# dedis/kyber

Hardware: AMD Instinct MI355X
Metric: scalar-muls/s + pairings/s per node; MSM sec at 2^20 points (higher is better)
Workload: dtype int32 limbs (radix 2^25.5), int64 accumulate; 1 GPU; Ed25519 batched fixed-base + var-base scalar-mul, 2^20 scalars per GPU (BASELINE.json configs[1]); elements_per_gpu=1048576

## Files before the change

kyber_amd/csrc/ed25519.hip:

```cpp
#ifndef KYB_TU_WAVES
#define KYB_TU_WAVES 2
#endif
#include "context.h"
#include "ed25519_dev.cuh"
#include "ed25519_launch.h"
#include "msm.cuh"
#include "ed25519_h2c.cuh"
#include <stdlib.h>
#include <string.h>

#include <algorithm>
#include <atomic>
#include <chrono>
#include <thread>
#include <vector>

namespace kyb {


template <int G = 2>
__global__ void ed25519_build_base_table_kernel(int32_t* __restrict__ tab, const uint32_t* __restrict__ point,
                                                uint32_t* __restrict__ ok, int rows = ED_TAB_POS * ED_TAB_ENT) {
    const int t = blockIdx.x * blockDim.x + threadIdx.x;
    if (t >= rows) return;
    ge_p3 B;
    if (point) {
        uint32_t pw[8];
        load_words8(pw, point);
        const bool good = ge_p3_fromwords(B, pw);
        if (t == 0) *ok = good ? 1u : 0u;
    } else {
        B.X = fe_bx(); B.Y = fe_by(); fe_1(B.Z); B.T = fe_bt();
    }
    ed_comb_row<G>(tab + (size_t)t * ED_TAB_STRIDE, t, B);
}

__global__ __launch_bounds__(64, KYB_TU_WAVES) void ed25519_encode_kernel(size_t n, const int32_t* __restrict__ proj,
                                                            const uint8_t* __restrict__ status,
                                                            uint32_t* __restrict__ out) {
    ed_encode_chunk(n, proj, (size_t)blockIdx.x * blockDim.x + threadIdx.x, [&](size_t i, uint32_t (&w)[8]) {
        if (status && status[i]) {
#pragma unroll
            for (int k = 0; k < 8; k++) w[k] = 0;
        }
        store_words8(out + i * 8, w);
    });
}


template <int G>
__global__ __launch_bounds__(256, 3) void ed25519_mul_base_kernel(
    size_t n, const uint32_t* __restrict__ scalars, uint32_t* __restrict__ out,
    const int32_t* __restrict__ tab, uint32_t flags, int32_t* __restrict__ proj) {
    const bool full = (flags & KYB_F_VARTIME) != 0;
    for (size_t idx = (size_t)blockIdx.x * blockDim.x + threadIdx.x; idx < n;
         idx += (size_t)gridDim.x * blockDim.x) {
        uint32_t a[8];
        load_words8(a, scalars + idx * 8);
        int8_t e[65];
        recode16(e, a, full);
        ge_p3 h;
        ge_p3_0(h);
        ge_precomp t;
        ge_p1p1 r;
        const int npos = full ? EdComb<G>::POS : EdComb<G>::POS_CT;
        EdCombDigits<G> digits(e);
#pragma unroll 1
        for (int k = 0; k < npos; k++) {
            const int d = digits.next(k);
            if (full && __ballot(d != 0) == 0) continue;
            select_precomp_tab<EdComb<G>::ENT>(t, tab, k, d);
            ge_madd(r, h, t);
            ge_p1p1_to_p3(h, r);
        }
        if (proj) {
            store_proj(proj, idx, h);
            continue;
        }
        uint32_t w[8];
// ... 26 lines not shown
        for (int l = 0; l < 10; l++) {
            t.ypx.v[l] ^= (t.ypx.v[l] ^ w[l]) & keep;
            t.ymx.v[l] ^= (t.ymx.v[l] ^ w[10 + l]) & keep;
            t.xy2d.v[l] ^= (t.xy2d.v[l] ^ w[20 + l]) & keep;
        }
    }
    ge_precomp_cneg(t, neg);
}
__global__ __launch_bounds__(256, 3) void ed25519_mul_base_uniform_kernel(
    size_t n, const uint32_t* __restrict__ scalars, uint32_t* __restrict__ out,
    const int32_t* __restrict__ tab, int32_t* __restrict__ proj) {
    for (size_t idx = (size_t)blockIdx.x * blockDim.x + threadIdx.x; idx < n;
         idx += (size_t)gridDim.x * blockDim.x) {
        uint32_t a[8];
        load_words8(a, scalars + idx * 8);
        int8_t e[65];
        recode16(e, a, false);
        ge_p3 h;
        ge_p3_0(h);
        ge_precomp t;
        ge_p1p1 r;
        EdCombDigits<1> digits(e);
#pragma unroll 1
        for (int i = 0; i < 64; i++) {
            select_precomp_uniform(t, tab, i, digits.next(i));
            ge_madd(r, h, t);
            ge_p1p1_to_p3(h, r);
        }
        if (proj) {
            store_proj(proj, idx, h);
            continue;
        }
        uint32_t w[8];
        ge_p3_towords(w, h);
        store_words8(out + idx * 8, w);
    }
}


template <bool GTAB, bool UNI = false>
__global__ __launch_bounds__(128, 3) void ed25519_mul_kernel(
    size_t n, const uint32_t* __restrict__ scalars, const uint32_t* __restrict__ points,
    size_t points_stride, uint32_t* __restrict__ out, uint8_t* __restrict__ status,
    uint32_t flags, int32_t* __restrict__ proj, int4* __restrict__ gtab) {
    const size_t idx = (size_t)blockIdx.x * blockDim.x + threadIdx.x;
    if (idx >= n) return;
    const bool full = !UNI && (flags & KYB_F_VARTIME) != 0;
    uint32_t pw[8], a[8];
    load_words8(pw, points + idx * points_stride);
    load_words8(a, scalars + idx * 8);
    ge_p3 A;
    const bool ok = ge_p3_fromwords(A, pw);
    int8_t e[65];
    recode16(e, a, full);
    ge_p3 h;
    const int vt_top = full ? wave_top_digit(a) : 63;
    if constexpr (GTAB) {
        TabGlobal tab{gtab + idx * 80};
        ge_scalarmult_w4<UNI, true>(h, e, A, full, tab, vt_top);
    } else {
        TabScratch tab;
        ge_scalarmult_w4<UNI, true>(h, e, A, full, tab, vt_top);
    }
    if (proj) {
        store_proj(proj, idx, h);
        if (status) status[idx] = ok ? KYB_ST_OK : KYB_ST_BAD_POINT;
        return;
    }
    uint32_t w[8];
    ge_p3_towords(w, h);
    if (!ok) {
#pragma unroll
        for (int i = 0; i < 8; i++) w[i] = 0;
    }
    store_words8(out + idx * 8, w);
    if (status) status[idx] = ok ? KYB_ST_OK : KYB_ST_BAD_POINT;
}

int ed25519_build_tables(DeviceCtx* ctx) {
    KYB_HIP_CHECK(hipMalloc(&ctx->ed_base_tab, ED_TAB_WORDS * sizeof(int32_t)));
    hipLaunchKernelGGL(ed25519_build_base_table_kernel<2>, dim3((ED_TAB_POS * ED_TAB_ENT + 63) / 64), dim3(64), 0,
                       nullptr, ctx->ed_base_tab, (const uint32_t*)nullptr, (uint32_t*)nullptr, ED_TAB_POS * ED_TAB_ENT);
    KYB_HIP_CHECK(hipGetLastError());
    const auto t0 = std::chrono::steady_clock::now();
    KYB_HIP_CHECK(hipMalloc(&ctx->ed_wide_tab, ED_WIDE_WORDS * sizeof(int32_t)));
    hipLaunchKernelGGL(ed25519_build_base_table_kernel<ED_COMB_G>, dim3((EdWide::ROWS + 63) / 64), dim3(64), 0, nullptr,
                       ctx->ed_wide_tab, (const uint32_t*)nullptr, (uint32_t*)nullptr, EdWide::ROWS);
    KYB_HIP_CHECK(hipGetLastError());
    KYB_HIP_CHECK(hipStreamSynchronize(nullptr));
    ctx->ed_wide_build_us = std::chrono::duration_cast<std::chrono::microseconds>(std::chrono::steady_clock::now() - t0).count();
    return KYB_OK;
}
void ed25519_free_tables(DeviceCtx* ctx) {
    if (ctx->ed_base_tab) hipFree(ctx->ed_base_tab);
    if (ctx->ed_wide_tab) hipFree(ctx->ed_wide_tab);
    ctx->ed_base_tab = ctx->ed_wide_tab = nullptr;
}

constexpr size_t ENC_DEFER_MIN = 4096;


static int launch_mul_base(DeviceCtx* ctx, size_t n, const void* d_scalars, void* d_out, uint32_t flags,
                           hipStream_t st, const int32_t* tab = nullptr) {
    const bool wide = !tab && !(flags & KYB_F_UNIFORM);
    if (!tab) tab = wide ? ctx->ed_wide_tab : ctx->ed_base_tab;
    if (n == 0) return KYB_OK;
    const int block = 256;
    size_t want = (n + block - 1) / block;
    size_t cap = (size_t)ctx->num_cu * 8;
    int grid = (int)(want < cap ? want : cap);
    EdSlab w{};
    std::lock_guard<std::recursive_mutex> enq_lock(ctx->enq_mu);
    if (n >= ENC_DEFER_MIN)
        if (int rc = ed_slab(ctx, st, ED_SLAB_MUL_BASE, n, &w)) return rc;
    if (flags & KYB_F_UNIFORM) {
        hipLaunchKernelGGL(ed25519_mul_base_uniform_kernel, dim3(grid), dim3(block), 0, st, n,
                           (const uint32_t*)d_scalars, (uint32_t*)d_out, tab, w.proj);
    } else {
        const auto kernel = wide ? ed25519_mul_base_kernel<ED_COMB_G> : ed25519_mul_base_kernel<2>;
        hipLaunchKernelGGL(kernel, dim3(grid), dim3(block), 0, st, n, (const uint32_t*)d_scalars, (uint32_t*)d_out, tab,
                           flags, w.proj);
    }
    if (w.proj)
        hipLaunchKernelGGL(ed25519_encode_kernel, ed_encode_grid(n), dim3(ED_ENC_BLOCK), 0, st, n, w.proj,
                           (const uint8_t*)nullptr, (uint32_t*)d_out);
    KYB_HIP_CHECK(hipGetLastError());
    return KYB_OK;
}
static int launch_mul(size_t n, const void* d_scalars, const void* d_points, size_t stride, void* d_out,
                      void* d_status, uint32_t flags, hipStream_t st) {
    if (n == 0) return KYB_OK;
    const int block = 128;
    size_t grid = (n + block - 1) / block;
    EdSlab w{};
    uint8_t* stat = (uint8_t*)d_status;
    DeviceCtx* ctx;
    int rc = get_ctx(&ctx);
    if (rc) return rc;
    std::lock_guard<std::recursive_mutex> enq_lock(ctx->enq_mu);
    const bool defer = n >= ENC_DEFER_MIN, uni = (flags & KYB_F_UNIFORM) != 0;
    const auto kernel = defer ? (uni ? ed25519_mul_kernel<true, true> : ed25519_mul_kernel<true, false>)
                              : (uni ? ed25519_mul_kernel<false, true> : ed25519_mul_kernel<false, false>);
    if (defer) {
        if ((rc = ed_slab(ctx, st, ed_slab_mul(stat == nullptr), n, &w))) return rc;
        if (!stat) stat = w.status;
    }
    hipLaunchKernelGGL(kernel, dim3((unsigned)grid), dim3(block), 0, st, n, (const uint32_t*)d_scalars,
                       (const uint32_t*)d_points, stride, (uint32_t*)d_out, stat, flags, w.proj, w.gtab);
    if (w.proj)
        hipLaunchKernelGGL(ed25519_encode_kernel, ed_encode_grid(n), dim3(ED_ENC_BLOCK), 0, st, n, w.proj,
                           (const uint8_t*)stat, (uint32_t*)d_out);
    KYB_HIP_CHECK(hipGetLastError());
    return KYB_OK;
}

}

using namespace kyb;

static bool ed_mul_flags_bad(uint32_t flags) {
    return (flags & ~(KYB_F_VARTIME | KYB_F_UNIFORM)) || (flags & (KYB_F_VARTIME | KYB_F_UNIFORM)) == (KYB_F_VARTIME | KYB_F_UNIFORM);
}

extern "C" {

int kyb_ed25519_mul_base_dev(size_t n, const void* d_scalars, void* d_out, uint32_t flags, void* stream) {
    if ((n && (!d_scalars || !d_out)) || ed_mul_flags_bad(flags)) {
        set_error("kyb_ed25519_mul_base_dev: bad argument");
        return KYB_E_ARG;
    }
    DeviceCtx* ctx;
    int rc = get_ctx(&ctx);
    if (rc) return rc;
    return launch_mul_base(ctx, n, d_scalars, d_out, flags, (hipStream_t)stream);
}

int kyb_ed25519_mul_dev(size_t n, const void* d_scalars, const void* d_points, void* d_out, void* d_status,
                        uint32_t flags, void* stream) {
    if ((n && (!d_scalars || !d_points || !d_out)) || ed_mul_flags_bad(flags)) {
        set_error("kyb_ed25519_mul_dev: bad argument");
        return KYB_E_ARG;
    }
    DeviceCtx* ctx;
    int rc = get_ctx(&ctx);
// ... 498 lines not shown
```

kyber_amd/csrc/ed25519_dev.cuh:

```cuda
#pragma once
#include "ge25519.cuh"

#if !defined(__HIPCC__)
#include <type_traits>
struct int4 { int32_t x, y, z, w; };
struct uint4 { uint32_t x, y, z, w; };
inline int4 make_int4(int32_t x, int32_t y, int32_t z, int32_t w) { return int4{x, y, z, w}; }
inline uint4 make_uint4(uint32_t x, uint32_t y, uint32_t z, uint32_t w) { return uint4{x, y, z, w}; }
#define KYB_DEV_CONST static
#else
#define KYB_DEV_CONST __device__
#endif

namespace kyb {

constexpr int ED_TAB_POS = 33;
constexpr int ED_TAB_ENT = 136;
constexpr int ED_TAB_STRIDE = 32;
constexpr int ED_TAB_WORDS = ED_TAB_POS * ED_TAB_ENT * ED_TAB_STRIDE;

template <int G>
struct EdComb {
    static constexpr int POS = (65 + G - 1) / G;
    static constexpr int POS_CT = (64 + G - 1) / G;
// ... 13 lines not shown
    const uint4 b = reinterpret_cast<const uint4*>(p)[1];
    w[0] = a.x; w[1] = a.y; w[2] = a.z; w[3] = a.w;
    w[4] = b.x; w[5] = b.y; w[6] = b.z; w[7] = b.w;
}
KYB_DEV void store_words8(uint32_t* __restrict__ p, const uint32_t w[8]) {
    reinterpret_cast<uint4*>(p)[0] = make_uint4(w[0], w[1], w[2], w[3]);
    reinterpret_cast<uint4*>(p)[1] = make_uint4(w[4], w[5], w[6], w[7]);
}

template <int G>
KYB_DEV void ed_comb_row(int32_t* __restrict__ o, int t, const ge_p3& B) {
    constexpr int ENT = EdComb<G>::ENT;
    const int pos = t / ENT, j = t - pos * ENT;
    ge_cached cB;
    ge_p3_to_cached(cB, B);
    ge_p3 acc;
    ge_p3_0(acc);
    ge_p1p1 r;
#pragma unroll 1
    for (int bit = 4 * G - 1; bit >= 0; bit--) {
        ge_dbl(r, acc.X, acc.Y, acc.Z);
        ge_p1p1_to_p3(acc, r);
        if (((j + 1) >> bit) & 1) {
            ge_add(r, acc, cB);
            ge_p1p1_to_p3(acc, r);
        }
    }
#pragma unroll 1
    for (int k = 0; k < 4 * G * pos; k++) {
        ge_dbl(r, acc.X, acc.Y, acc.Z);
        ge_p1p1_to_p3(acc, r);
    }
    fe zi, x, y, ypx, ymx, xy2d, z;
    fe_invert(zi, acc.Z);
    fe_mul(x, acc.X, zi);
    fe_mul(y, acc.Y, zi);
    fe_add(ypx, y, x);
    fe_sub(ymx, y, x);
    fe_mul(xy2d, x, y);
    fe_mul(xy2d, xy2d, fe_d2());
    fe_1(z);
    fe_mul(ypx, ypx, z);
    fe_mul(ymx, ymx, z);
#pragma unroll
    for (int l = 0; l < 10; l++) {
        o[l] = ypx.v[l];
        o[10 + l] = ymx.v[l];
        o[20 + l] = xy2d.v[l];
    }
    o[30] = o[31] = 0;
}

constexpr int ENC_CHUNK = 16;

KYB_DEV void store_proj(int32_t* __restrict__ proj, size_t idx, const ge_p3& h) {
    int32_t* o = proj + idx * 30;
#pragma unroll
    for (int l = 0; l < 10; l++) {
        o[l] = h.X.v[l];
        o[10 + l] = h.Y.v[l];
        o[20 + l] = h.Z.v[l];
    }
}
KYB_DEV void load_fe(fe& f, const int32_t* __restrict__ p) {
#pragma unroll
    for (int l = 0; l < 10; l++) f.v[l] = p[l];
}
template <class Emit>
KYB_DEV void ed_encode_chunk(size_t n, const int32_t* __restrict__ proj, size_t lane, Emit emit) {
    const size_t lo = lane * ENC_CHUNK;
    if (lo >= n) return;
    const int cnt = (int)((n - lo) < (size_t)ENC_CHUNK ? (n - lo) : (size_t)ENC_CHUNK);
    fe pre[ENC_CHUNK];
    fe z, acc;
    load_fe(acc, proj + lo * 30 + 20);
    pre[0] = acc;
#pragma unroll 1
    for (int j = 1; j < cnt; j++) {
        load_fe(z, proj + (lo + j) * 30 + 20);
        fe_mul(acc, acc, z);
        pre[j] = acc;
    }
    fe inv;
    fe_invert(inv, acc);
#pragma unroll 1
    for (int j = cnt - 1; j >= 0; j--) {
        fe zi, X, Y;
        load_fe(z, proj + (lo + j) * 30 + 20);
        if (j > 0) {
            fe_mul(zi, inv, pre[j - 1]);
            fe_mul(inv, inv, z);
        } else {
            zi = inv;
        }
        load_fe(X, proj + (lo + j) * 30);
        load_fe(Y, proj + (lo + j) * 30 + 10);
        uint32_t w[8];
        ge_encode_with_zinv(w, X, Y, zi);
        emit(lo + j, w);
    }
}

template <int ENT>
KYB_DEV void select_precomp_tab(ge_precomp& t, const int32_t* __restrict__ tab, int pos, int b) {
    const bool neg = b < 0;
    const int babs = neg ? -b : b;
    const int4* e = reinterpret_cast<const int4*>(tab + (size_t)(pos * ENT + (babs ? babs - 1 : 0)) * ED_TAB_STRIDE);
    int32_t w[32];
#pragma unroll
    for (int i = 0; i < 8; i++) {
        const int4 x = e[i];
        w[4 * i] = x.x;
        w[4 * i + 1] = x.y;
        w[4 * i + 2] = x.z;
        w[4 * i + 3] = x.w;
    }
#pragma unroll
    for (int l = 0; l < 10; l++) {
        t.ypx.v[l] = w[l];
        t.ymx.v[l] = w[10 + l];
        t.xy2d.v[l] = w[20 + l];
    }
    if (babs == 0) {
        fe_1(t.ypx);
        fe_1(t.ymx);
        fe_0(t.xy2d);
    }
    ge_precomp_cneg(t, neg);
}

KYB_DEV void ed_pack_digits(uint32_t pk[8], const int8_t e[65]) {
#pragma unroll
// ... 241 lines not shown
```

kyber_amd/csrc/ed25519_ring.cuh:

```cuda
#pragma once
#include "ed25519_dleq.cuh"

namespace kyb {

KYB_HD void blake2xb_root_iv_keyed(uint64_t (&h)[8], uint32_t keylen) {
    constexpr uint64_t IV[8] = KYB_BLAKE2B_IV;
#pragma unroll
    for (int i = 0; i < 8; i++) h[i] = IV[i];
    h[0] ^= 0x01010040ull | ((uint64_t)keylen << 8);
    h[1] ^= 0xffffffff00000000ull;
}

struct EdRingMid {
    uint64_t h[8];
    uint64_t t;
    uint64_t r;
    uint32_t czero[8];
    uint64_t buf[32];
};
static_assert(sizeof(EdRingMid) == 368, "ed25519_launch.h: ED_SLAB_RING parks 5 x 120 B per lane, this at byte 128");

struct EdRingPrefix {
    const uint8_t* msg;
    size_t len;
// ... 123 lines not shown
    TabGlobal t{tab};
    ge_window_table(t, A);
    return ok;
}

KYB_DEV int ed_ring_step(uint32_t (&c)[8], const uint32_t sw[8], bool full, bool linkable, const EdRingShared& sh,
                         const int4* tx, const EdRingLaneMem& mem) {
    int8_t es[65], ec[65];
    recode16(es, sw, full);
    recode16(ec, c, full);
    int vt_top = 63;
    if (full) {
        const int ta = wave_top_digit(sw), tb = wave_top_digit(c);
        vt_top = ta > tb ? ta : tb;
    }
    const int8_t l63 = es[63], l64 = es[64];
    const bool drop = (int)l63 + 16 * (int)l64 > 8;
    ge_p3 h;
    const int sides = linkable ? 2 : 1;
#pragma unroll 1
    for (int side = 0; side < sides; side++) {
        es[63] = (side == 0 && drop) ? (int8_t)0 : l63;
        es[64] = (side == 0 && drop) ? (int8_t)0 : l64;
        TabGlobal tp{const_cast<int4*>(sh.tabs + (side ? ED_RING_TAB_LINK : ED_RING_TAB_G) * 80)};
        TabGlobal tq{const_cast<int4*>(side ? mem.tag_tab : tx)};
        ge_double_scalarmult_w4(h, es, ec, full, tp, tq, vt_top);
        if (side + 1 < sides) store_proj(mem.park, 0, h);
    }
    uint32_t pg[8], ph[8];
    if (linkable) {
        fe zg, zz, inv, zi;
        load_fe(zg, mem.park + 20);
        fe_mul(zz, zg, h.Z);
        fe_invert(inv, zz);
        fe_mul(zi, inv, zg);
        ge_encode_with_zinv(ph, h.X, h.Y, zi);
        fe_mul(zi, inv, h.Z);
        load_fe(h.X, mem.park);
        load_fe(h.Y, mem.park + 10);
        ge_encode_with_zinv(pg, h.X, h.Y, zi);
    } else {
        ge_p3_towords(pg, h);
#pragma unroll
        for (int i = 0; i < 8; i++) ph[i] = 0;
    }
    return ed_ring_finish(c, mem.mid, pg, ph, linkable);
}

struct EdRingSig {
    size_t ring;
    const uint32_t* keys;
    const uint32_t* sig;
    const uint8_t* msg;
    size_t len;
    const uint8_t* scope;
    size_t scope_len;
};

KYB_DEV int ed_ring_lane(uint32_t (&c)[8], const EdRingSig& s, size_t start, size_t steps, bool full, const EdRingShared& sh,
                         const EdRingLaneMem& mem) {
    const bool linkable = s.scope != nullptr;
    bool bad = false, exhausted = false;
    {
        uint32_t tw[8], tc[8];
        if (linkable) {
            load_words8(tw, s.sig + 8 * (1 + s.ring));
            ed_canon_point_bytes(tc, tw);
// ... 54 lines not shown
```

kyber_amd/csrc/fe25519.cuh:

```cuda
#pragma once
#include "hd.h"

namespace kyb {

struct fe {
    int32_t v[10];
#if defined(KYB_FE_AUDIT)
    double mag = 2.0;
#endif
};

#if defined(KYB_FE_AUDIT)
inline double& fe_audit_max() {
    static double m = 0;
    return m;
}
inline double& fe_audit_max19() {
    static double m = 0;
    return m;
}
inline void fe_audit_note(double pf, double pg, double scale) {
    const double x = pf * pg * scale;
    if (x > fe_audit_max()) fe_audit_max() = x;
    if (pg > fe_audit_max19()) fe_audit_max19() = pg;
// ... 259 lines not shown
        h[i] -= c << w_;
    }
    h[9] &= (1 << 25) - 1;
    uint32_t u[10];
#pragma unroll
    for (int i = 0; i < 10; i++) u[i] = (uint32_t)h[i];
    w[0] = u[0] | (u[1] << 26);
    w[1] = (u[1] >> 6) | (u[2] << 19);
    w[2] = (u[2] >> 13) | (u[3] << 13);
    w[3] = (u[3] >> 19) | (u[4] << 6);
    w[4] = u[5] | (u[6] << 25);
    w[5] = (u[6] >> 7) | (u[7] << 19);
    w[6] = (u[7] >> 13) | (u[8] << 12);
    w[7] = (u[8] >> 20) | (u[9] << 6);
}
KYB_DEV void fe_fromwords(fe& h, const uint32_t w[8]) {
    h.v[0] = (int32_t)(w[0] & 0x3ffffff);
    h.v[1] = (int32_t)(((w[0] >> 26) | (w[1] << 6)) & 0x1ffffff);
    h.v[2] = (int32_t)(((w[1] >> 19) | (w[2] << 13)) & 0x3ffffff);
    h.v[3] = (int32_t)(((w[2] >> 13) | (w[3] << 19)) & 0x1ffffff);
    h.v[4] = (int32_t)((w[3] >> 6) & 0x3ffffff);
    h.v[5] = (int32_t)(w[4] & 0x1ffffff);
    h.v[6] = (int32_t)(((w[4] >> 25) | (w[5] << 7)) & 0x3ffffff);
    h.v[7] = (int32_t)(((w[5] >> 19) | (w[6] << 13)) & 0x1ffffff);
    h.v[8] = (int32_t)(((w[6] >> 12) | (w[7] << 20)) & 0x3ffffff);
    h.v[9] = (int32_t)((w[7] >> 6) & 0x1ffffff);
    KYB_FE_MAG_SET(h, 2.0);
}
KYB_DEV bool fe_isnegative(const fe& f) {
    uint32_t w[8];
    fe_towords(w, f);
    return w[0] & 1;
}
KYB_DEV bool fe_isnonzero(const fe& f) {
    uint32_t w[8];
    fe_towords(w, f);
    uint32_t r = 0;
#pragma unroll
    for (int i = 0; i < 8; i++) r |= w[i];
    return r != 0;
}

}
```

kyber_amd/csrc/ge25519.cuh:

```cuda
#pragma once
#include "fe25519.cuh"

namespace kyb {

struct ge_p2 { fe X, Y, Z; };
struct ge_p3 { fe X, Y, Z, T; };
struct ge_p1p1 { fe X, Y, Z, T; };
struct ge_cached { fe YpX, YmX, Z, T2d; };
struct ge_precomp { fe ypx, ymx, xy2d; };

#include "ed25519_consts.inc"

KYB_DEV void ge_p3_0(ge_p3& h) {
    fe_0(h.X);
    fe_1(h.Y);
    fe_1(h.Z);
    fe_0(h.T);
}
KYB_DEV void ge_cached_0(ge_cached& c) {
    fe_1(c.YpX);
    fe_1(c.YmX);
    fe_1(c.Z);
    fe_0(c.T2d);
}
// ... 43 lines not shown
KYB_DEV void ge_madd(ge_p1p1& r, const ge_p3& p, const ge_precomp& q) {
    fe t0;
    fe_add(r.X, p.Y, p.X);
    fe_sub(r.Y, p.Y, p.X);
    fe_mul(r.Z, r.X, q.ypx);
    fe_mul(r.Y, r.Y, q.ymx);
    fe_mul(r.T, q.xy2d, p.T);
    fe_add(t0, p.Z, p.Z);
    fe_sub(r.X, r.Z, r.Y);
    fe_add(r.Y, r.Z, r.Y);
    fe_add(r.Z, t0, r.T);
    fe_sub(r.T, t0, r.T);
}
KYB_DEV void ge_cached_cneg(ge_cached& c, bool neg) {
    fe_cswap(c.YpX, c.YmX, neg);
    fe nt;
    fe_neg(nt, c.T2d);
    fe_cmov(c.T2d, nt, neg);
}
KYB_DEV void ge_precomp_cneg(ge_precomp& c, bool neg) {
    fe_cswap(c.ypx, c.ymx, neg);
    fe nt;
    fe_neg(nt, c.xy2d);
    fe_cmov(c.xy2d, nt, neg);
}

KYB_DEV void ge_encode_with_zinv(uint32_t w[8], const fe& X, const fe& Y, const fe& zinv) {
    fe x, y;
    fe_mul(x, X, zinv);
    fe_mul(y, Y, zinv);
    fe_towords(w, y);
    w[7] ^= (uint32_t)fe_isnegative(x) << 31;
}
KYB_DEV void ge_p3_towords(uint32_t w[8], const ge_p3& p) {
    fe zi;
    fe_invert(zi, p.Z);
    ge_encode_with_zinv(w, p.X, p.Y, zi);
}
KYB_DEV bool ge_p3_fromwords(ge_p3& p, const uint32_t w[8]) {
    fe u, v, v3, vxx, check;
    fe_fromwords(p.Y, w);
    fe_1(p.Z);
    fe_sq(u, p.Y);
    fe_mul(v, u, fe_d());
    fe_sub(u, u, p.Z);
    fe_add(v, v, p.Z);
    fe_sq(v3, v);
    fe_mul(v3, v3, v);
    fe_sq(p.X, v3);
    fe_mul(p.X, p.X, v);
    fe_mul(p.X, p.X, u);
    fe_pow22523(p.X, p.X);
    fe_mul(p.X, p.X, v3);
    fe_mul(p.X, p.X, u);
    fe_sq(vxx, p.X);
    fe_mul(vxx, vxx, v);
    fe_sub(check, vxx, u);
    bool ok = true;
    if (fe_isnonzero(check)) {
        fe_add(check, vxx, u);
        ok = !fe_isnonzero(check);
        fe xs;
        fe_mul(xs, p.X, fe_sqrtm1());
        p.X = xs;
    }
    const bool sign = (w[7] >> 31) != 0;
    fe nx;
    fe_neg(nx, p.X);
    fe_cmov(p.X, nx, fe_isnegative(p.X) != sign);
// ... 52 lines not shown
```

kyber_amd/csrc/ed25519_dleq.hip:

```cpp
#ifndef KYB_TU_WAVES
#define KYB_TU_WAVES 2
#endif
#include "context.h"
#include "ed25519_dleq.cuh"
#include "ed25519_launch.h"

namespace kyb {

static_assert(ED_ST_OK == KYB_ST_OK && ED_ST_BAD_POINT == KYB_ST_BAD_POINT && ED_ST_DLEQ_CHALLENGE == KYB_ST_DLEQ_CHALLENGE &&
                  ED_ST_PICK_EXHAUSTED == KYB_ST_PICK_EXHAUSTED,
              "status values of include/kyber_hip.h");

__global__ __launch_bounds__(128, 3) void ed25519_dleq_challenge_kernel(
    size_t n, const uint32_t* __restrict__ xG, const uint32_t* __restrict__ xH, const uint32_t* __restrict__ vG,
    const uint32_t* __restrict__ vH, uint32_t* __restrict__ c, uint8_t* __restrict__ status) {
    const size_t i = (size_t)blockIdx.x * blockDim.x + threadIdx.x;
    if (i >= n) return;
    uint32_t a[8], b[8], u[8], v[8], cw[8];
    load_words8(a, xG + i * 8);
    load_words8(b, xH + i * 8);
    load_words8(u, vG + i * 8);
    load_words8(v, vH + i * 8);
    const int draws = ed_dleq_challenge(cw, a, b, u, v);
    store_words8(c + i * 8, cw);
// ... 7 lines not shown
    const uint32_t* __restrict__ expect, uint32_t flags, int32_t* __restrict__ proj, uint8_t* __restrict__ st,
    int4* __restrict__ gtab) {
    const size_t lane = (size_t)blockIdx.x * blockDim.x + threadIdx.x;
    const size_t idx = lane < n ? lane : n - 1;
    uint32_t cw[8], rw[8];
    load_words8(cw, C + idx * 8);
    int s;
    {
        uint32_t a[8], b[8], u[8], v[8];
        const bool fs = (flags & KYB_F_DLEQ_FS) != 0;
        if (fs) {
            load_words8(a, xG + idx * 8);
            load_words8(b, xH + idx * 8);
            load_words8(u, VG + idx * 8);
            load_words8(v, VH + idx * 8);
        }
        s = ed_dleq_challenge_status(cw, expect, fs, a, b, u, v);
    }
    load_words8(rw, R + idx * 8);
    TabGlobal tp{gtab + lane * 160}, tq{gtab + lane * 160 + 80};
    const bool live = lane < n;
    s = ed_dleq_lane(
        s, cw, rw, (flags & KYB_F_VARTIME) != 0, tp, tq,
        [&](int side, uint32_t(&pw)[8], uint32_t(&qw)[8]) {
            load_words8(pw, side ? H + idx * hs : G + idx * gs);
            load_words8(qw, (side ? xH : xG) + idx * 8);
        },
        [&](int side, const ge_p3& h) {
            if (live) store_proj(proj, 2 * idx + side, h);
        });
    if (live) st[idx] = (uint8_t)s;
}

__global__ __launch_bounds__(64, KYB_TU_WAVES) void ed25519_dleq_encode_kernel(
    size_t n, const int32_t* __restrict__ proj, const uint8_t* __restrict__ st, const uint32_t* __restrict__ VG,
    const uint32_t* __restrict__ VH, uint8_t* __restrict__ ok, uint8_t* __restrict__ status) {
    static_assert(ENC_CHUNK % 2 == 0, "a and b of one proof share a chunk");
    bool b_same = false;
    ed_encode_chunk(2 * n, proj, (size_t)blockIdx.x * blockDim.x + threadIdx.x, [&](size_t i, uint32_t(&w)[8]) {
        const size_t e = i >> 1;
        uint32_t v[8], cv[8];
        load_words8(v, ((i & 1) ? VH : VG) + e * 8);
        ed_canon_point_bytes(cv, v);
        const bool same = ed_words8_equal(cv, w);
        if (i & 1) {
            b_same = same;
        } else {
            const uint8_t s = st[e];
            ok[e] = (s == KYB_ST_OK && same && b_same) ? 1 : 0;
            if (status) status[e] = s;
        }
    });
}

static int launch_challenge(size_t n, const void* xG, const void* xH, const void* vG, const void* vH, void* c, void* status,
                            hipStream_t st) {
    DeviceCtx* ctx;
    const int rc = get_ctx(&ctx);
    if (rc) return rc;
    for (size_t lo = 0; lo < n; lo += ED_PIECE) {
        const size_t cnt = std::min(ED_PIECE, n - lo);
        hipLaunchKernelGGL(ed25519_dleq_challenge_kernel, dim3((unsigned)((cnt + 127) / 128)), dim3(128), 0, st, cnt,
                           (const uint32_t*)xG + lo * 8, (const uint32_t*)xH + lo * 8, (const uint32_t*)vG + lo * 8,
                           (const uint32_t*)vH + lo * 8, (uint32_t*)c + lo * 8, status ? (uint8_t*)status + lo : nullptr);
        KYB_HIP_CHECK(hipGetLastError());
    }
    return KYB_OK;
}

struct DleqArgs {
    const void *G, *H, *xG, *xH, *C, *R, *VG, *VH, *expect;
    size_t g_stride, h_stride;
// ... 101 lines not shown
```

kyber_amd/csrc/ed25519_launch.h:

```cpp
#pragma once
#include "context.h"
#include "ed25519_dev.cuh"

namespace kyb {

constexpr size_t ED_PIECE = size_t(1) << 18;
constexpr size_t ED_TAB_BLOCK = 128;

constexpr size_t ED_TAB_BYTES = sizeof(TabScratch);
constexpr size_t ED_PROJ_LIMBS = 3 * sizeof(fe) / sizeof(int32_t);
static_assert(ED_TAB_BYTES == 80 * sizeof(int4) && ED_TAB_BYTES == 1280, "TabGlobal: 8 x 10 int4 per lane and table");
static_assert(ED_PROJ_LIMBS == 30, "store_proj / ed_encode_chunk: 30 limbs per parked point");

struct EdSlabDesc {
    size_t tabs, parked;
    bool status, whole_blocks;
};
struct EdSlab {
    int4* gtab;
    int32_t* proj;
    uint8_t* status;
};
constexpr size_t ed_slab_lanes(const EdSlabDesc& d, size_t lanes) {
    return d.whole_blocks ? (lanes + ED_TAB_BLOCK - 1) / ED_TAB_BLOCK * ED_TAB_BLOCK : lanes;
// ... 18 lines not shown
              "the parked point, then the midstate, inside the lane's five slots");
static_assert(ed_slab_bytes(ED_SLAB_VERIFY, 1) == ED_TAB_BLOCK * 1401 + 256 && ed_slab_lanes(ED_SLAB_DLEQ, 129) == 256, "whole blocks");
static_assert(ed_slab_bytes(ed_slab_mul(false), 4099) == 4099 * 1400 + 256 && ed_slab_bytes(ed_slab_mul(true), 4099) == 4099 * 1401 + 256 &&
                  ed_slab_bytes(ED_SLAB_MUL_BASE, 4099) == 4099 * 120 + 256,
              "unrounded");

inline int ed_slab(DeviceCtx* ctx, hipStream_t st, const EdSlabDesc& d, size_t lanes, EdSlab* s) {
    void* base;
    if (int rc = ctx_workspace(ctx, WS_ED, st, ed_slab_bytes(d, lanes), &base)) return rc;
    lanes = ed_slab_lanes(d, lanes);
    const size_t tab_bytes = lanes * d.tabs * ED_TAB_BYTES, proj_bytes = lanes * d.parked * ED_PROJ_LIMBS * sizeof(int32_t);
    s->gtab = (int4*)base;
    s->proj = (int32_t*)((uint8_t*)base + tab_bytes);
    s->status = d.status ? (uint8_t*)base + tab_bytes + proj_bytes : nullptr;
    return KYB_OK;
}

template <class F>
int ed_for_pieces(size_t n, hipStream_t st, const EdSlabDesc& d, F&& enqueue) {
    DeviceCtx* ctx;
    int rc = get_ctx(&ctx);
    if (rc) return rc;
    std::lock_guard<std::recursive_mutex> enq_lock(ctx->enq_mu);
    for (size_t lo = 0; lo < n; lo += ED_PIECE) {
        EdSlab slab;
        if ((rc = ed_slab(ctx, st, d, std::min(ED_PIECE, n), &slab))) return rc;
        enqueue(ctx, lo, std::min(ED_PIECE, n - lo), slab);
        KYB_HIP_CHECK(hipGetLastError());
    }
    return KYB_OK;
}

constexpr unsigned ED_ENC_BLOCK = 64;
inline dim3 ed_encode_grid(size_t points) {
    const size_t lanes = (points + ENC_CHUNK - 1) / ENC_CHUNK;
    return dim3((unsigned)((lanes + ED_ENC_BLOCK - 1) / ED_ENC_BLOCK));
}

}
```

kyber_amd/csrc/ed25519_verify.hip:

```cpp
#ifndef KYB_TU_WAVES
#define KYB_TU_WAVES 2
#endif
#include "context.h"
#include "ed25519_verify.cuh"
#include "ed25519_launch.h"

#include <vector>

namespace kyb {

static_assert(ED_ST_OK == KYB_ST_OK && ED_ST_BAD_POINT == KYB_ST_BAD_POINT &&
                  ED_ST_SIG_NONCANONICAL == KYB_ST_SIG_NONCANONICAL && ED_ST_SIG_SMALL_ORDER == KYB_ST_SIG_SMALL_ORDER,
              "status values of include/kyber_hip.h");

__global__ __launch_bounds__(128, 3) void ed25519_verify_kernel(
    size_t n, const uint32_t* __restrict__ pubs, const uint8_t* __restrict__ msgs, const uint64_t* __restrict__ off,
    const uint32_t* __restrict__ sigs, const int32_t* __restrict__ wide, sf::Mod m, int32_t* __restrict__ proj,
    uint8_t* __restrict__ st, int4* __restrict__ gtab) {
    const size_t lane = (size_t)blockIdx.x * blockDim.x + threadIdx.x;
    const size_t idx = lane < n ? lane : n - 1;
    uint32_t aw[8], rw[8], sw[8];
    load_words8(aw, pubs + idx * 8);
    load_words8(rw, sigs + idx * 16);
    load_words8(sw, sigs + idx * 16 + 8);
    const uint64_t lo = off[idx], hi = off[idx + 1];
    const size_t len = hi >= lo ? (size_t)(hi - lo) : 0;
    TabGlobal tab{gtab + lane * 80};
    ge_p3 T;
    const int s = ed_verify_lane(T, rw, sw, aw, msgs + lo, len, wide, m, tab);
    if (lane >= n) return;
    store_proj(proj, idx, T);
    st[idx] = (uint8_t)s;
}
__global__ __launch_bounds__(64, KYB_TU_WAVES) void ed25519_verify_encode_kernel(
    size_t n, const int32_t* __restrict__ proj, const uint8_t* __restrict__ st, const uint32_t* __restrict__ sigs,
    uint8_t* __restrict__ ok, uint8_t* __restrict__ status) {
    ed_encode_chunk(n, proj, (size_t)blockIdx.x * blockDim.x + threadIdx.x, [&](size_t i, uint32_t (&w)[8]) {
        uint32_t r[8];
        load_words8(r, sigs + i * 16);
        uint32_t diff = 0;
#pragma unroll
        for (int k = 0; k < 8; k++) diff |= r[k] ^ w[k];
        const uint8_t s = st[i];
        ok[i] = (s == KYB_ST_OK && diff == 0) ? 1 : 0;
        if (status) status[i] = s;
    });
}

__global__ __launch_bounds__(128, 3) void ed25519_mul2_kernel(
    size_t n, const uint32_t* __restrict__ a, const uint32_t* __restrict__ P, const uint32_t* __restrict__ b,
    const uint32_t* __restrict__ Q, uint32_t flags, int32_t* __restrict__ proj, uint8_t* __restrict__ st,
    int4* __restrict__ gtab) {
    const size_t lane = (size_t)blockIdx.x * blockDim.x + threadIdx.x;
    const size_t idx = lane < n ? lane : n - 1;
    uint32_t aw[8], pw[8], bw[8], qw[8];
    load_words8(aw, a + idx * 8);
    load_words8(pw, P + idx * 8);
    load_words8(bw, b + idx * 8);
    load_words8(qw, Q + idx * 8);
    TabGlobal tp{gtab + lane * 160}, tq{gtab + lane * 160 + 80};
    ge_p3 h;
    const bool ok = ed_mul2_lane(h, aw, pw, bw, qw, (flags & KYB_F_VARTIME) != 0, tp, tq);
    if (lane >= n) return;
    store_proj(proj, idx, h);
    st[idx] = ok ? KYB_ST_OK : KYB_ST_BAD_POINT;
}
__global__ __launch_bounds__(64, KYB_TU_WAVES) void ed25519_mul2_encode_kernel(
    size_t n, const int32_t* __restrict__ proj, const uint8_t* __restrict__ st, uint32_t* __restrict__ out,
    uint8_t* __restrict__ status) {
    ed_encode_chunk(n, proj, (size_t)blockIdx.x * blockDim.x + threadIdx.x, [&](size_t i, uint32_t (&w)[8]) {
        const uint8_t s = st[i];
        if (s) {
#pragma unroll
            for (int k = 0; k < 8; k++) w[k] = 0;
        }
        store_words8(out + i * 8, w);
        if (status) status[i] = s;
    });
}

static const sf::Mod& ed_order() {
    static const sf::Mod m = sf::make_mod(sf::Q_ED25519, false);
    return m;
}

static int launch_verify(size_t n, const void* d_pubs, const void* d_msgs, const void* d_off, const void* d_sigs,
                         void* d_ok, void* d_status, hipStream_t st) {
    return ed_for_pieces(n, st, ED_SLAB_VERIFY, [&](DeviceCtx* ctx, size_t lo, size_t cnt, const EdSlab& w) {
        const uint32_t* sigs = (const uint32_t*)d_sigs + lo * 16;
        hipLaunchKernelGGL(ed25519_verify_kernel, dim3((unsigned)((cnt + 127) / 128)), dim3(128), 0, st, cnt,
                           (const uint32_t*)d_pubs + lo * 8, (const uint8_t*)d_msgs, (const uint64_t*)d_off + lo, sigs,
                           (const int32_t*)ctx->ed_wide_tab, ed_order(), w.proj, w.status, w.gtab);
        hipLaunchKernelGGL(ed25519_verify_encode_kernel, ed_encode_grid(cnt), dim3(ED_ENC_BLOCK), 0, st, cnt,
                           (const int32_t*)w.proj, (const uint8_t*)w.status, sigs, (uint8_t*)d_ok + lo,
                           d_status ? (uint8_t*)d_status + lo : nullptr);
    });
}

static int launch_mul2(size_t n, const void* d_a, const void* d_P, const void* d_b, const void* d_Q, void* d_out,
                       void* d_status, uint32_t flags, hipStream_t st) {
    return ed_for_pieces(n, st, ED_SLAB_MUL2, [&](DeviceCtx*, size_t lo, size_t cnt, const EdSlab& w) {
        hipLaunchKernelGGL(ed25519_mul2_kernel, dim3((unsigned)((cnt + 127) / 128)), dim3(128), 0, st, cnt,
                           (const uint32_t*)d_a + lo * 8, (const uint32_t*)d_P + lo * 8, (const uint32_t*)d_b + lo * 8,
// ... 96 lines not shown
```

Baseline: 176.2 million scalar-muls/s.

## Replace Fermat field inversion with batched safegcd divsteps inversion

Swaps the exponentiation-based fe_invert for a Bernstein–Yang style divsteps inversion on 30-bit limbs, used in encoding, batch-inversion chunks, ring finalization and table building. Non-uniform callers may exit the batch loop early once a whole wave has g equal to zero. Uniform/constant-time paths pass a fixed flag to run all 20 batches. This aims to cut the roughly 255 squarings per inversion, at the cost of int64 multiply-heavy matrix updates and added complexity.

Result: no change. 178.0 million scalar-muls/s, median of 6 (+1.0%).

```diff
diff --git a/kyber_amd/csrc/ed25519.hip b/kyber_amd/csrc/ed25519.hip
--- a/kyber_amd/csrc/ed25519.hip
+++ b/kyber_amd/csrc/ed25519.hip
@@ -37,14 +37,14 @@
 
 __global__ __launch_bounds__(64, KYB_TU_WAVES) void ed25519_encode_kernel(size_t n, const int32_t* __restrict__ proj,
                                                             const uint8_t* __restrict__ status,
-                                                            uint32_t* __restrict__ out) {
+                                                            uint32_t* __restrict__ out, uint32_t uniform) {
     ed_encode_chunk(n, proj, (size_t)blockIdx.x * blockDim.x + threadIdx.x, [&](size_t i, uint32_t (&w)[8]) {
         if (status && status[i]) {
 #pragma unroll
             for (int k = 0; k < 8; k++) w[k] = 0;
         }
         store_words8(out + i * 8, w);
-    });
+    }, uniform != 0);
 }
 
 
@@ -137,7 +137,7 @@
             continue;
         }
         uint32_t w[8];
-        ge_p3_towords(w, h);
+        ge_p3_towords(w, h, true);
         store_words8(out + idx * 8, w);
     }
 }
@@ -173,7 +173,7 @@
         return;
     }
     uint32_t w[8];
-    ge_p3_towords(w, h);
+    ge_p3_towords(w, h, UNI);
     if (!ok) {
 #pragma unroll
         for (int i = 0; i < 8; i++) w[i] = 0;
@@ -228,7 +228,7 @@
     }
     if (w.proj)
         hipLaunchKernelGGL(ed25519_encode_kernel, ed_encode_grid(n), dim3(ED_ENC_BLOCK), 0, st, n, w.proj,
-                           (const uint8_t*)nullptr, (uint32_t*)d_out);
+                           (const uint8_t*)nullptr, (uint32_t*)d_out, (flags & KYB_F_UNIFORM) ? 1u : 0u);
     KYB_HIP_CHECK(hipGetLastError());
     return KYB_OK;
 }
@@ -254,7 +254,7 @@
                        (const uint32_t*)d_points, stride, (uint32_t*)d_out, stat, flags, w.proj, w.gtab);
     if (w.proj)
         hipLaunchKernelGGL(ed25519_encode_kernel, ed_encode_grid(n), dim3(ED_ENC_BLOCK), 0, st, n, w.proj,
-                           (const uint8_t*)stat, (uint32_t*)d_out);
+                           (const uint8_t*)stat, (uint32_t*)d_out, uni ? 1u : 0u);
     KYB_HIP_CHECK(hipGetLastError());
     return KYB_OK;
 }
diff --git a/kyber_amd/csrc/ed25519_dev.cuh b/kyber_amd/csrc/ed25519_dev.cuh
--- a/kyber_amd/csrc/ed25519_dev.cuh
+++ b/kyber_amd/csrc/ed25519_dev.cuh
@@ -69,7 +69,7 @@
         ge_p1p1_to_p3(acc, r);
     }
     fe zi, x, y, ypx, ymx, xy2d, z;
-    fe_invert(zi, acc.Z);
+    fe_invert_divsteps(zi, acc.Z);
     fe_mul(x, acc.X, zi);
     fe_mul(y, acc.Y, zi);
     fe_add(ypx, y, x);
@@ -104,7 +104,7 @@
     for (int l = 0; l < 10; l++) f.v[l] = p[l];
 }
 template <class Emit>
-KYB_DEV void ed_encode_chunk(size_t n, const int32_t* __restrict__ proj, size_t lane, Emit emit) {
+KYB_DEV void ed_encode_chunk(size_t n, const int32_t* __restrict__ proj, size_t lane, Emit emit, bool fixed = false) {
     const size_t lo = lane * ENC_CHUNK;
     if (lo >= n) return;
     const int cnt = (int)((n - lo) < (size_t)ENC_CHUNK ? (n - lo) : (size_t)ENC_CHUNK);
@@ -119,7 +119,7 @@
         pre[j] = acc;
     }
     fe inv;
-    fe_invert(inv, acc);
+    fe_invert_divsteps(inv, acc, fixed);
 #pragma unroll 1
     for (int j = cnt - 1; j >= 0; j--) {
         fe zi, X, Y;
diff --git a/kyber_amd/csrc/ed25519_ring.cuh b/kyber_amd/csrc/ed25519_ring.cuh
--- a/kyber_amd/csrc/ed25519_ring.cuh
+++ b/kyber_amd/csrc/ed25519_ring.cuh
@@ -179,7 +179,7 @@
         fe zg, zz, inv, zi;
         load_fe(zg, mem.park + 20);
         fe_mul(zz, zg, h.Z);
-        fe_invert(inv, zz);
+        fe_invert_divsteps(inv, zz);
         fe_mul(zi, inv, zg);
         ge_encode_with_zinv(ph, h.X, h.Y, zi);
         fe_mul(zi, inv, h.Z);
diff --git a/kyber_amd/csrc/fe25519.cuh b/kyber_amd/csrc/fe25519.cuh
--- a/kyber_amd/csrc/fe25519.cuh
+++ b/kyber_amd/csrc/fe25519.cuh
@@ -315,6 +315,139 @@
     fe_towords(w, f);
     return w[0] & 1;
 }
+
+constexpr int FE_DIVSTEPS_BATCHES = 20;
+constexpr uint32_t fe_p_inv32() {
+    const uint32_t p0 = 0u - 19u;
+    uint32_t x = p0;
+    for (int k = 0; k < 5; k++) x *= 2u - p0 * x;
+    return x;
+}
+constexpr int32_t fe_p_limb30(int i) { return i == 0 ? (1 << 30) - 19 : i < 8 ? (1 << 30) - 1 : (1 << 15) - 1; }
+KYB_DEV int fe_invert_divsteps_counted(fe& out, const fe& z, bool fixed) {
+    constexpr int NL = 9;
+    constexpr uint32_t M30 = (1u << 30) - 1;
+    constexpr uint32_t PINV = fe_p_inv32();
+    uint32_t w[8];
+    fe_towords(w, z);
+    int32_t f[NL], g[NL], d[NL], e[NL];
+#pragma unroll
+    for (int i = 0; i < NL; i++) {
+        const int bit = 30 * i, idx = bit >> 5, sh = bit & 31;
+        uint32_t x = w[idx] >> sh;
+        if (sh > 2 && idx + 1 < 8) x |= w[idx + 1] << (32 - sh);
+        g[i] = (int32_t)(x & M30);
+        f[i] = fe_p_limb30(i);
+        d[i] = 0;
+        e[i] = 0;
+    }
+    e[0] = 1;
+    int32_t eta = -1;
+    int batches = 0;
+#pragma unroll 1
+    for (; batches < FE_DIVSTEPS_BATCHES; batches++) {
+        if (!fixed) {
+            uint32_t gnz = 0;
+#pragma unroll
+            for (int i = 0; i < NL; i++) gnz |= (uint32_t)g[i];
+#if defined(__HIP_DEVICE_COMPILE__)
+            if (__ballot(gnz != 0) == 0) break;
+#else
+            if (!gnz) break;
+#endif
+        }
+        uint32_t f0 = (uint32_t)f[0] | ((uint32_t)f[1] << 30), g0 = (uint32_t)g[0] | ((uint32_t)g[1] << 30);
+        uint32_t u = 1, v = 0, q = 0, rr = 1;
+#pragma unroll 6
+        for (int k = 0; k < 30; k++) {
+            const uint32_t c1 = (uint32_t)(eta >> 31);
+            const uint32_t c2 = 0u - (g0 & 1u);
+            const uint32_t x = (f0 ^ c1) - c1, y = (u ^ c1) - c1, t = (v ^ c1) - c1;
+            g0 += x & c2;
+            q += y & c2;
+            rr += t & c2;
+            const uint32_t sw = c1 & c2;
+            eta = (int32_t)(((uint32_t)eta ^ sw) - 1u);
+            f0 += g0 & sw;
+            u += q & sw;
+            v += rr & sw;
+            g0 >>= 1;
+            u <<= 1;
+            v <<= 1;
+        }
+        const int32_t U = (int32_t)u, V = (int32_t)v, Q = (int32_t)q, R = (int32_t)rr;
+        {
+            int64_t cf = (int64_t)U * f[0] + (int64_t)V * g[0], cg = (int64_t)Q * f[0] + (int64_t)R * g[0];
+            cf >>= 30;
+            cg >>= 30;
+#pragma unroll
+            for (int i = 1; i < NL; i++) {
+                cf += (int64_t)U * f[i] + (int64_t)V * g[i];
+                cg += (int64_t)Q * f[i] + (int64_t)R * g[i];
+                f[i - 1] = (int32_t)((uint32_t)cf & M30);
+                g[i - 1] = (int32_t)((uint32_t)cg & M30);
+                cf >>= 30;
+                cg >>= 30;
+            }
+            f[NL - 1] = (int32_t)cf;
+            g[NL - 1] = (int32_t)cg;
+        }
+        {
+            const int32_t sd = d[NL - 1] >> 31, se = e[NL - 1] >> 31;
+            int32_t md = (U & sd) + (V & se), me = (Q & sd) + (R & se);
+            int64_t cd = (int64_t)U * d[0] + (int64_t)V * e[0], ce = (int64_t)Q * d[0] + (int64_t)R * e[0];
+            md -= (int32_t)((PINV * (uint32_t)cd + (uint32_t)md) & M30);
+            me -= (int32_t)((PINV * (uint32_t)ce + (uint32_t)me) & M30);
+            cd -= (int64_t)19 * md;
+            ce -= (int64_t)19 * me;
+            cd >>= 30;
+            ce >>= 30;
+#pragma unroll
+            for (int i = 1; i < NL; i++) {
+                cd += (int64_t)U * d[i] + (int64_t)V * e[i];
+                ce += (int64_t)Q * d[i] + (int64_t)R * e[i];
+                if (i == NL - 1) {
+                    cd += (int64_t)md * (1 << 15);
+                    ce += (int64_t)me * (1 << 15);
+                }
+                d[i - 1] = (int32_t)((uint32_t)cd & M30);
+                e[i - 1] = (int32_t)((uint32_t)ce & M30);
+                cd >>= 30;
+                ce >>= 30;
+            }
+            d[NL - 1] = (int32_t)cd;
+            e[NL - 1] = (int32_t)ce;
+        }
+    }
+    const int32_t sf = f[NL - 1] >> 31;
+    {
+        int32_t neg = d[NL - 1] >> 31;
+        int64_t c = 0;
+#pragma unroll
+        for (int i = 0; i < NL; i++) {
+            c += (int64_t)(((d[i] + (fe_p_limb30(i) & neg)) ^ sf) - sf);
+            d[i] = i + 1 < NL ? (int32_t)((uint32_t)c & M30) : (int32_t)c;
+            c >>= 30;
+        }
+        neg = d[NL - 1] >> 31;
+        c = 0;
+#pragma unroll
+        for (int i = 0; i < NL; i++) {
+            c += (int64_t)d[i] + (int64_t)(fe_p_limb30(i) & neg);
+            d[i] = i + 1 < NL ? (int32_t)((uint32_t)c & M30) : (int32_t)c;
+            c >>= 30;
+        }
+    }
+#pragma unroll
+    for (int k = 0; k < 8; k++) {
+        const int bit = 32 * k, idx = bit / 30, sh = bit - 30 * idx;
+        uint32_t x = (uint32_t)d[idx] >> sh;
+        w[k] = x | ((uint32_t)d[idx + 1] << (30 - sh));
+    }
+    fe_fromwords(out, w);
+    return batches;
+}
+KYB_DEV void fe_invert_divsteps(fe& out, const fe& z, bool fixed = false) { (void)fe_invert_divsteps_counted(out, z, fixed); }
 KYB_DEV bool fe_isnonzero(const fe& f) {
     uint32_t w[8];
     fe_towords(w, f);
diff --git a/kyber_amd/csrc/ge25519.cuh b/kyber_amd/csrc/ge25519.cuh
--- a/kyber_amd/csrc/ge25519.cuh
+++ b/kyber_amd/csrc/ge25519.cuh
@@ -99,9 +99,9 @@
     fe_towords(w, y);
     w[7] ^= (uint32_t)fe_isnegative(x) << 31;
 }
-KYB_DEV void ge_p3_towords(uint32_t w[8], const ge_p3& p) {
+KYB_DEV void ge_p3_towords(uint32_t w[8], const ge_p3& p, bool fixed = false) {
     fe zi;
-    fe_invert(zi, p.Z);
+    fe_invert_divsteps(zi, p.Z, fixed);
     ge_encode_with_zinv(w, p.X, p.Y, zi);
 }
 KYB_DEV bool ge_p3_fromwords(ge_p3& p, const uint32_t w[8]) {
```

## Interleave encode chunk points across lanes and move prefix products to LDS

Applied to the files above, without the earlier changes.

The batched-inversion encode kernels now take points strided across the block instead of giving each lane a contiguous run of 16. Neighbouring lanes therefore read neighbouring projective records, which is meant to coalesce the global loads and stores. The main encode kernel also keeps the running prefix products in a column-major LDS buffer rather than a per-thread register/scratch array, to cut register pressure and scratch spills. The DLEQ path groups record pairs so a proof's two points stay together. The cost is extra LDS use per block and more complex indexing.

After: 169.4 million scalar-muls/s before, 172.9 million scalar-muls/s after, median of 6. 1.02x the previous value.

```diff
diff --git a/kyber_amd/csrc/ed25519.hip b/kyber_amd/csrc/ed25519.hip
--- a/kyber_amd/csrc/ed25519.hip
+++ b/kyber_amd/csrc/ed25519.hip
@@ -35,10 +35,14 @@
     ed_comb_row<G>(tab + (size_t)t * ED_TAB_STRIDE, t, B);
 }
 
-__global__ __launch_bounds__(64, KYB_TU_WAVES) void ed25519_encode_kernel(size_t n, const int32_t* __restrict__ proj,
+__global__ __launch_bounds__(ED_ENC_BLOCK, KYB_TU_WAVES) void ed25519_encode_kernel(size_t n, const int32_t* __restrict__ proj,
                                                             const uint8_t* __restrict__ status,
                                                             uint32_t* __restrict__ out) {
-    ed_encode_chunk(n, proj, (size_t)blockIdx.x * blockDim.x + threadIdx.x, [&](size_t i, uint32_t (&w)[8]) {
+    __shared__ int32_t pre_lds[EncPreLds<ED_ENC_BLOCK>::WORDS];
+    static_assert(ED_ENC_BLOCK % 64 == 0 && sizeof(pre_lds) <= 80 * 1024 && sizeof(pre_lds) / (ED_ENC_BLOCK / 64) * 4 <= 160 * 1024,
+                  "LDS: at least two blocks on a CU, and a wave on every SIMD");
+    EncPreLds<ED_ENC_BLOCK> pre{pre_lds + threadIdx.x};
+    ed_encode_chunk(n, proj, ed_encode_first(), blockDim.x, pre, [&](size_t i, uint32_t (&w)[8]) {
         if (status && status[i]) {
 #pragma unroll
             for (int k = 0; k < 8; k++) w[k] = 0;
diff --git a/kyber_amd/csrc/ed25519_dev.cuh b/kyber_amd/csrc/ed25519_dev.cuh
--- a/kyber_amd/csrc/ed25519_dev.cuh
+++ b/kyber_amd/csrc/ed25519_dev.cuh
@@ -103,38 +103,67 @@
 #pragma unroll
     for (int l = 0; l < 10; l++) f.v[l] = p[l];
 }
-template <class Emit>
-KYB_DEV void ed_encode_chunk(size_t n, const int32_t* __restrict__ proj, size_t lane, Emit emit) {
-    const size_t lo = lane * ENC_CHUNK;
-    if (lo >= n) return;
-    const int cnt = (int)((n - lo) < (size_t)ENC_CHUNK ? (n - lo) : (size_t)ENC_CHUNK);
+struct EncPreScratch {
     fe pre[ENC_CHUNK];
+    KYB_DEV void put(int j, const fe& f) { pre[j] = f; }
+    KYB_DEV void get(fe& f, int j) const { f = pre[j]; }
+};
+template <int LANES>
+struct EncPreLds {
+    int32_t* col;
+    static constexpr int WORDS = ENC_CHUNK * 10 * LANES;
+    KYB_DEV void put(int j, const fe& f) {
+#pragma unroll
+        for (int l = 0; l < 10; l++) col[(j * 10 + l) * LANES] = f.v[l];
+    }
+    KYB_DEV void get(fe& f, int j) const {
+#pragma unroll
+        for (int l = 0; l < 10; l++) f.v[l] = col[(j * 10 + l) * LANES];
+        KYB_FE_MAG_SET(f, 1.01);
+    }
+};
+#if defined(__HIPCC__)
+template <int GROUP = 1>
+KYB_DEV size_t ed_encode_first() {
+    return (size_t)blockIdx.x * blockDim.x * (ENC_CHUNK / GROUP) + threadIdx.x;
+}
+#endif
+template <int GROUP = 1, class Pre, class Emit>
+KYB_DEV void ed_encode_chunk(size_t n, const int32_t* __restrict__ proj, size_t first, size_t stride, Pre& pre, Emit emit) {
+    static_assert(GROUP >= 1 && ENC_CHUNK % GROUP == 0, "whole records per lane");
+    int cnt = 0;
+#pragma unroll
+    for (int r = 0; r < ENC_CHUNK / GROUP; r++) cnt += (first + r * stride < n) ? GROUP : 0;
+    if (cnt == 0) return;
+    auto point = [&](int j) { return (first + (size_t)(j / GROUP) * stride) * GROUP + (size_t)(j % GROUP); };
     fe z, acc;
-    load_fe(acc, proj + lo * 30 + 20);
-    pre[0] = acc;
+    load_fe(acc, proj + point(0) * 30 + 20);
+    pre.put(0, acc);
 #pragma unroll 1
     for (int j = 1; j < cnt; j++) {
-        load_fe(z, proj + (lo + j) * 30 + 20);
+        load_fe(z, proj + point(j) * 30 + 20);
         fe_mul(acc, acc, z);
-        pre[j] = acc;
+        pre.put(j, acc);
     }
     fe inv;
     fe_invert(inv, acc);
 #pragma unroll 1
     for (int j = cnt - 1; j >= 0; j--) {
+        const size_t i = point(j);
         fe zi, X, Y;
-        load_fe(z, proj + (lo + j) * 30 + 20);
+        load_fe(z, proj + i * 30 + 20);
         if (j > 0) {
-            fe_mul(zi, inv, pre[j - 1]);
+            pre.get(zi, j - 1);
+            fe_mul(zi, inv, zi);
             fe_mul(inv, inv, z);
         } else {
             zi = inv;
         }
-        load_fe(X, proj + (lo + j) * 30);
-        load_fe(Y, proj + (lo + j) * 30 + 10);
+        load_fe(X, proj + i * 30);
+        load_fe(Y, proj + i * 30 + 10);
         uint32_t w[8];
         ge_encode_with_zinv(w, X, Y, zi);
-        emit(lo + j, w);
+        emit(i, w);
     }
 }
 
diff --git a/kyber_amd/csrc/ed25519_dleq.hip b/kyber_amd/csrc/ed25519_dleq.hip
--- a/kyber_amd/csrc/ed25519_dleq.hip
+++ b/kyber_amd/csrc/ed25519_dleq.hip
@@ -63,12 +63,13 @@
     if (live) st[idx] = (uint8_t)s;
 }
 
-__global__ __launch_bounds__(64, KYB_TU_WAVES) void ed25519_dleq_encode_kernel(
+__global__ __launch_bounds__(ED_ENC_BLOCK, KYB_TU_WAVES) void ed25519_dleq_encode_kernel(
     size_t n, const int32_t* __restrict__ proj, const uint8_t* __restrict__ st, const uint32_t* __restrict__ VG,
     const uint32_t* __restrict__ VH, uint8_t* __restrict__ ok, uint8_t* __restrict__ status) {
     static_assert(ENC_CHUNK % 2 == 0, "a and b of one proof share a chunk");
     bool b_same = false;
-    ed_encode_chunk(2 * n, proj, (size_t)blockIdx.x * blockDim.x + threadIdx.x, [&](size_t i, uint32_t(&w)[8]) {
+    EncPreScratch pre;
+    ed_encode_chunk<2>(n, proj, ed_encode_first<2>(), blockDim.x, pre, [&](size_t i, uint32_t(&w)[8]) {
         const size_t e = i >> 1;
         uint32_t v[8], cv[8];
         load_words8(v, ((i & 1) ? VH : VG) + e * 8);
diff --git a/kyber_amd/csrc/ed25519_launch.h b/kyber_amd/csrc/ed25519_launch.h
--- a/kyber_amd/csrc/ed25519_launch.h
+++ b/kyber_amd/csrc/ed25519_launch.h
@@ -74,9 +74,6 @@
 }
 
 constexpr unsigned ED_ENC_BLOCK = 64;
-inline dim3 ed_encode_grid(size_t points) {
-    const size_t lanes = (points + ENC_CHUNK - 1) / ENC_CHUNK;
-    return dim3((unsigned)((lanes + ED_ENC_BLOCK - 1) / ED_ENC_BLOCK));
+constexpr size_t ED_ENC_SPAN = size_t(ED_ENC_BLOCK) * ENC_CHUNK;
+inline dim3 ed_encode_grid(size_t points) { return dim3((unsigned)((points + ED_ENC_SPAN - 1) / ED_ENC_SPAN)); }
 }
-
-}
diff --git a/kyber_amd/csrc/ed25519_verify.hip b/kyber_amd/csrc/ed25519_verify.hip
--- a/kyber_amd/csrc/ed25519_verify.hip
+++ b/kyber_amd/csrc/ed25519_verify.hip
@@ -32,10 +32,11 @@
     store_proj(proj, idx, T);
     st[idx] = (uint8_t)s;
 }
-__global__ __launch_bounds__(64, KYB_TU_WAVES) void ed25519_verify_encode_kernel(
+__global__ __launch_bounds__(ED_ENC_BLOCK, KYB_TU_WAVES) void ed25519_verify_encode_kernel(
     size_t n, const int32_t* __restrict__ proj, const uint8_t* __restrict__ st, const uint32_t* __restrict__ sigs,
     uint8_t* __restrict__ ok, uint8_t* __restrict__ status) {
-    ed_encode_chunk(n, proj, (size_t)blockIdx.x * blockDim.x + threadIdx.x, [&](size_t i, uint32_t (&w)[8]) {
+    EncPreScratch pre;
+    ed_encode_chunk(n, proj, ed_encode_first(), blockDim.x, pre, [&](size_t i, uint32_t (&w)[8]) {
         uint32_t r[8];
         load_words8(r, sigs + i * 16);
         uint32_t diff = 0;
@@ -65,10 +66,11 @@
     store_proj(proj, idx, h);
     st[idx] = ok ? KYB_ST_OK : KYB_ST_BAD_POINT;
 }
-__global__ __launch_bounds__(64, KYB_TU_WAVES) void ed25519_mul2_encode_kernel(
+__global__ __launch_bounds__(ED_ENC_BLOCK, KYB_TU_WAVES) void ed25519_mul2_encode_kernel(
     size_t n, const int32_t* __restrict__ proj, const uint8_t* __restrict__ st, uint32_t* __restrict__ out,
     uint8_t* __restrict__ status) {
-    ed_encode_chunk(n, proj, (size_t)blockIdx.x * blockDim.x + threadIdx.x, [&](size_t i, uint32_t (&w)[8]) {
+    EncPreScratch pre;
+    ed_encode_chunk(n, proj, ed_encode_first(), blockDim.x, pre, [&](size_t i, uint32_t (&w)[8]) {
         const uint8_t s = st[i];
         if (s) {
 #pragma unroll
```
